# educating-dip/diffusion_models_dev_project

Hardware: NVIDIA B200
Metric: SCD samples/sec at 256^2 (higher is better)
Workload: dtype f32

## Files before the change

bench_support/adm_unet.py:

```python
import math

import torch
import torch.nn as nn
import torch.nn.functional as F


def sinusoidal_embedding(t, dim, max_period=10000.0):
    half = dim // 2
    freqs = torch.exp(-math.log(max_period) * torch.arange(half, dtype=torch.float32, device=t.device) / half)
    args = t[:, None].float() * freqs[None]
    return torch.cat([torch.cos(args), torch.sin(args)], dim=-1)


def _norm(ch):
    return nn.GroupNorm(32, ch)


def _small_init(conv, std=0.02):
    nn.init.normal_(conv.weight, std=std)
    nn.init.zeros_(conv.bias)
    return conv


class Res(nn.Module):
    def __init__(self, cin, cout, emb_ch, resample=None):
        super().__init__()
        self.resample = resample
        self.n1 = _norm(cin)
        self.c1 = nn.Conv2d(cin, cout, 3, padding=1)
        self.emb = nn.Linear(emb_ch, 2 * cout)
        self.n2 = _norm(cout)
        self.c2 = _small_init(nn.Conv2d(cout, cout, 3, padding=1))
        self.skip = nn.Identity() if cin == cout else nn.Conv2d(cin, cout, 1)

    def _rs(self, v):
        if self.resample == 'up':
            return F.interpolate(v, scale_factor=2, mode='nearest')
        if self.resample == 'down':
            return F.avg_pool2d(v, 2)
        return v

    def forward(self, x, emb):
        h = F.silu(self.n1(x))
        if self.resample is not None:
            h, x = self._rs(h), self._rs(x)
        h = self.c1(h)
        scale, shift = self.emb(F.silu(emb))[:, :, None, None].chunk(2, dim=1)
        h = self.n2(h) * (1 + scale) + shift
        h = self.c2(F.silu(h))
        return self.skip(x) + h


class Attn(nn.Module):
    def __init__(self, ch, head_ch):
        super().__init__()
        self.heads = ch // head_ch
        self.norm = _norm(ch)
        self.qkv = nn.Conv1d(ch, 3 * ch, 1)
        self.proj = _small_init(nn.Conv1d(ch, ch, 1))

    def forward(self, x, emb=None):
        b, c, hh, ww = x.shape
        q, k, v = self.qkv(self.norm(x).reshape(b, c, -1)).reshape(b * self.heads, 3 * c // self.heads, -1).chunk(3, dim=1)
        a = F.scaled_dot_product_attention(q.transpose(1, 2), k.transpose(1, 2), v.transpose(1, 2))
        a = a.transpose(1, 2).reshape(b, c, -1)
        return x + self.proj(a).reshape(b, c, hh, ww)


class Stage(nn.ModuleList):
    def forward(self, x, emb):
        for m in self:
            x = m(x, emb)
        return x


class AdmUNet(nn.Module):
    def __init__(self, image_size=256, in_channels=1, model_channels=256, out_channels=2,
                 num_res_blocks=1, channel_mult=(1, 1, 2, 2, 4, 4), attention_resolutions=(16,),
                 num_head_channels=64, max_period=1e4):
        super().__init__()
        ch = model_channels
        emb_ch = 4 * ch
        self.model_channels = ch
        self.max_period = max_period
        self.out_channels = out_channels
        self.time = nn.Sequential(nn.Linear(ch, emb_ch), nn.SiLU(), nn.Linear(emb_ch, emb_ch))
        attn_ds = {image_size // r for r in attention_resolutions}
        self.stem = nn.Conv2d(in_channels, ch, 3, padding=1)
        self.down = nn.ModuleList()
        skips = [ch]
        cur, ds = ch, 1
        for level, mult in enumerate(channel_mult):
            for _ in range(num_res_blocks):
                blk = [Res(cur, mult * ch, emb_ch)]
                cur = mult * ch
                if ds in attn_ds:
                    blk.append(Attn(cur, num_head_channels))
                self.down.append(Stage(blk)); skips.append(cur)
            if level != len(channel_mult) - 1:
                self.down.append(Stage([Res(cur, cur, emb_ch, 'down')])); skips.append(cur)
                ds *= 2
        self.mid = Stage([Res(cur, cur, emb_ch), Attn(cur, num_head_channels), Res(cur, cur, emb_ch)])
        self.up = nn.ModuleList()
        for level, mult in list(enumerate(channel_mult))[::-1]:
            for i in range(num_res_blocks + 1):
                blk = [Res(cur + skips.pop(), mult * ch, emb_ch)]
                cur = mult * ch
                if ds in attn_ds:
                    blk.append(Attn(cur, num_head_channels))
                if level and i == num_res_blocks:
                    blk.append(Res(cur, cur, emb_ch, 'up'))
                    ds //= 2
                self.up.append(Stage(blk))
        self.head = nn.Sequential(_norm(cur), nn.SiLU(), _small_init(nn.Conv2d(cur, out_channels, 3, padding=1)))

    def forward(self, x, timesteps):
        emb = self.time(sinusoidal_embedding(timesteps, self.model_channels, self.max_period))
        h = self.stem(x)
        hs = [h]
        for blk in self.down:
            h = blk(h, emb)
            hs.append(h)
        h = self.mid(h, emb)
        for blk in self.up:
            h = blk(torch.cat([h, hs.pop()], dim=1), emb)
        out = self.head(h)
        return out[:, :1] if self.out_channels == 2 else out


def small_unet():
    return AdmUNet(image_size=256, model_channels=32, out_channels=1, channel_mult=(1, 2, 4),
                   attention_resolutions=(16,), num_head_channels=32)


def aapm_unet():
    return AdmUNet()
```

diffusion_models_dev_project_b200/_lib.py:

```python
import ctypes as C
import os
import threading

_HERE = os.path.dirname(os.path.abspath(__file__))
LIB_PATH = os.environ.get("SCD_B200_LIB") or os.path.join(_HERE, "_lib", "libscd_b200.so")

SCD_E_INVALID = -10001
SCD_E_NODEVICE = -10002
SCD_E_WORKSPACE = -10003


class GeomDesc(C.Structure):
    _fields_ = [
        ("n0", C.c_int32), ("n1", C.c_int32),
        ("x_min", C.c_double), ("y_min", C.c_double), ("dx", C.c_double),
        ("n_angles", C.c_int32), ("angles", C.POINTER(C.c_double)),
        ("n_det", C.c_int32), ("s_min", C.c_double), ("ds", C.c_double),
        ("adj_scale", C.c_double),
    ]


_F = C.c_void_p
SIGNATURES = {
    "scd_geom_create": (C.c_int, [C.POINTER(GeomDesc), C.POINTER(C.c_void_p)]),
    "scd_geom_destroy": (C.c_int, [C.c_void_p]),
    "scd_fp_scratch_bytes": (C.c_size_t, [C.c_void_p, C.c_int]),
    "scd_fp": (C.c_int, [C.c_void_p, _F, _F, C.c_int, C.c_int, C.c_int, C.c_void_p, C.c_size_t, C.c_void_p]),
    "scd_bp_scratch_bytes": (C.c_size_t, [C.c_void_p, C.c_int]),
    "scd_bp": (C.c_int, [C.c_void_p, _F, _F, C.c_int, C.c_int, C.c_int, C.c_float, _F, C.c_float,
                         C.c_void_p, C.c_size_t, C.c_void_p]),
    "scd_sino_il_buffer_bytes": (C.c_size_t, [C.c_void_p, C.c_int]),
    "scd_fp_il": (C.c_int, [C.c_void_p, _F, _F, C.c_int, C.c_int, C.c_int, C.c_void_p, C.c_size_t, C.c_void_p]),
    "scd_bp_il": (C.c_int, [C.c_void_p, _F, _F, C.c_int, C.c_int, C.c_int, C.c_float, _F, C.c_float, C.c_void_p]),
    "scd_img_il_bytes": (C.c_size_t, [C.c_void_p, C.c_int]),
    "scd_img_il_pack": (C.c_int, [C.c_void_p, _F, _F, C.c_int, C.c_void_p]),
    "scd_img_il_unpack": (C.c_int, [C.c_void_p, _F, _F, C.c_int, C.c_void_p]),
    "scd_fp_ilimg": (C.c_int, [C.c_void_p, _F, _F, C.c_int, C.c_int, C.c_int, C.c_void_p]),
    "scd_bp_ilimg": (C.c_int, [C.c_void_p, _F, _F, C.c_int, C.c_int, C.c_int, C.c_float, _F, C.c_float, C.c_void_p]),
    "scd_cg_workspace_bytes": (C.c_size_t, [C.c_void_p, C.c_int]),
    "scd_cg": (C.c_int, [C.c_void_p, _F, _F, C.c_double, C.c_int, C.c_int, C.c_void_p, C.c_size_t, C.c_void_p]),
    "scd_tweedie_rhs": (C.c_int, [_F, _F, _F, _F, _F, C.c_int, C.c_double, _F, _F, C.c_int, C.c_int64, C.c_void_p]),
    "scd_ddim": (C.c_int, [_F, _F, _F, _F, _F, _F, C.c_int, C.c_double, _F, C.c_int, C.c_int64, C.c_void_p]),
    "scd_dds_step": (C.c_int, [C.c_void_p, _F, _F, _F, _F, _F, _F, _F, C.c_int, C.c_double, C.c_double,
                               C.c_int, _F, _F, C.c_int, C.c_void_p, C.c_size_t, C.c_void_p]),
    "scd_residual_sq_blocks": (C.c_int, [C.c_int64]),
    "scd_residual_sq": (C.c_int, [_F, _F, _F, _F, C.c_int64, C.c_void_p]),
    "scd_tv_blocks": (C.c_int, [C.c_int, C.c_int]),
    "scd_tv_loss": (C.c_int, [_F, _F, C.c_int, C.c_int, C.c_int, C.c_void_p]),
    "scd_tv_grad": (C.c_int, [_F, _F, C.c_int, C.c_int, C.c_int, C.c_void_p]),
    "scd_adapt_workspace_bytes": (C.c_size_t, [C.c_void_p, C.c_int, C.c_int]),
    "scd_adapt_fwd": (C.c_int, [C.c_void_p, _F, _F, _F, _F, _F, _F, C.c_int, C.c_double, C.c_int, C.c_int, C.c_double,
                                _F, _F, C.c_int, C.c_void_p, C.c_size_t, C.c_void_p]),
    "scd_adapt_bwd": (C.c_int, [C.c_void_p, _F, _F, _F, C.c_int, C.c_double, C.c_int, C.c_int, C.c_double, C.c_double,
                                _F, C.c_int, C.c_void_p, C.c_size_t, C.c_void_p]),
    "scd_ramp_filter": (C.c_int, [C.c_void_p, _F, _F, C.c_int, C.c_void_p]),
    "scd_bp_banded": (C.c_int, [C.c_void_p, _F, C.c_int, C.c_int, C.c_int, C.c_float, C.POINTER(C.c_void_p), C.c_int, C.c_int,
                                C.c_void_p, C.c_size_t, C.c_void_p]),
    "scd_bp_il_banded": (C.c_int, [C.c_void_p, _F, C.c_int, C.c_int, C.c_int, C.c_float, C.POINTER(C.c_void_p), C.c_int, C.c_int,
                                   C.c_void_p]),
    "scd_band_reduce": (C.c_int, [_F, C.c_int, C.c_int64, C.c_int, C.c_int, C.c_int, C.c_int, C.c_int, C.c_int,
                                  C.POINTER(C.c_void_p), C.c_int, C.c_int, _F, C.c_float, C.c_float, C.c_void_p]),
    "scd_fp_host": (C.c_int, [C.c_void_p, C.c_void_p, C.c_void_p, C.c_int]),
    "scd_bp_host": (C.c_int, [C.c_void_p, C.c_void_p, C.c_void_p, C.c_int]),
    "scd_geom_info": (C.c_int, [C.c_void_p, C.POINTER(C.c_int32), C.POINTER(C.c_int32),
                                C.POINTER(C.c_int32), C.POINTER(C.c_int32)]),
    "scd_launch_count": (C.c_int64, []),
    "scd_launch_count_reset": (None, []),
    "scd_set_tuning": (C.c_int, [C.c_void_p, C.c_char_p, C.c_int]),
    "scd_last_error_string": (C.c_char_p, []),
    "scd_version": (C.c_char_p, []),
}

_lib = None
_lock = threading.Lock()


def load():
    global _lib
    if _lib is not None:
        return _lib
    with _lock:
        if _lib is not None:
            return _lib
        if not os.path.exists(LIB_PATH):
            raise RuntimeError(
                f"{LIB_PATH} not found. Build it with `python -m diffusion_models_dev_project_b200.build` "
                "(needs nvcc). This package has no CPU or PyTorch fallback for the ray transform.")
        try:
            lib = C.CDLL(LIB_PATH)
        except OSError as e:
            raise RuntimeError(f"cannot load {LIB_PATH}: {e}") from e
        for name, (res, args) in SIGNATURES.items():
            fn = getattr(lib, name)
            fn.restype = res
            fn.argtypes = args
        _lib = lib
    return _lib


def last_error():
    s = load().scd_last_error_string()
    return s.decode() if s else ""


def check(rc, what):
    if rc != 0:
        raise RuntimeError(f"{what} failed (code {rc}): {last_error()}")
```

diffusion_models_dev_project_b200/build.py:

```python
import os
import shutil
import subprocess
import sys

HERE = os.path.dirname(os.path.abspath(__file__))
ROOT = os.path.dirname(HERE)
CSRC = os.path.join(HERE, "csrc")
LIB_DIR = os.path.join(HERE, "_lib")
LIB_PATH = os.path.join(LIB_DIR, "libscd_b200.so")
DEBUG_LIB_PATH = os.path.join(LIB_DIR, "libscd_b200_dbg.so")
SOURCES = ["geometry.cu", "fp_march.cu", "bp_tile.cu", "vec_ops.cu", "il_ops.cu", "loss_ops.cu", "adapt_ops.cu", "fbp_filter.cu", "cg_solver.cu", "peer_reduce.cu"]
HEADERS = [os.path.join(CSRC, "scd_internal.cuh"), os.path.join(ROOT, "include", "scd_b200.h")]
ARCH = ["-gencode", "arch=compute_100a,code=sm_100a"]


def _nvcc():
    cand = shutil.which("nvcc") or "/usr/local/cuda/bin/nvcc"
    if not os.path.exists(cand):
        raise RuntimeError("nvcc not found: libscd_b200.so cannot be built (there is no CPU fallback)")
    return cand


def needs_build(path=LIB_PATH):
    if not os.path.exists(path):
        return True
    t = os.path.getmtime(path)
    deps = [os.path.join(CSRC, s) for s in SOURCES] + HEADERS
    return any(os.path.getmtime(d) > t for d in deps)


def build(force=False, verbose=False, debug=False):
    out = DEBUG_LIB_PATH if debug else LIB_PATH
    if not force and not needs_build(out):
        return out
    os.makedirs(LIB_DIR, exist_ok=True)
    cmd = [_nvcc(), "-shared", "-Xcompiler", "-fPIC", "-O3", "-std=c++17", "-lineinfo", *ARCH,
           "-I", os.path.join(ROOT, "include"), "-I", CSRC]
    if debug:
        cmd += ["-DSCD_DEBUG_STAMPS"]
    if verbose:
        cmd += ["-Xptxas", "-v"]
    cmd += [os.path.join(CSRC, s) for s in SOURCES] + ["-o", out + ".tmp"]
    res = subprocess.run(cmd, capture_output=True, text=True)
    if res.returncode != 0:
        raise RuntimeError("nvcc failed:\n" + res.stdout + res.stderr)
    if verbose:
        sys.stderr.write(res.stdout + res.stderr)
    os.replace(out + ".tmp", out)
    return out


if __name__ == "__main__":
    p = build(force="--force" in sys.argv, verbose="--verbose" in sys.argv, debug="--debug" in sys.argv)
    print(p)
```

diffusion_models_dev_project_b200/fused.py:

```python
import ctypes as C

import torch
from torch import Tensor

from . import _lib


def _stream(device):
    return C.c_void_p(torch.cuda.current_stream(device).cuda_stream)


def _check_cuda_f32(**tensors):
    dev = None
    for name, t in tensors.items():
        if t is None:
            continue
        if not t.is_cuda:
            raise RuntimeError('%s must be a CUDA tensor (no CPU fallback in libscd_b200)' % name)
        if t.dtype != torch.float32:
            raise TypeError('%s must be float32, got %s' % (name, t.dtype))
        dev = dev or t.device
        if t.device != dev:
            raise ValueError('%s is on %s, expected %s' % (name, t.device, dev))
    return dev


def _times(t: Tensor, batch: int, device) -> Tensor:
    t = t.to(device=device, dtype=torch.float32).reshape(-1).contiguous()
    if t.numel() != batch:
        raise ValueError('time step tensor must have one entry per sample (%d != %d)' % (t.numel(), batch))
    return t


def tweedie_rhs(x: Tensor, s: Tensor, t: Tensor, abar: Tensor, atb: Tensor = None, gamma: float = 0.0):
    dev = _check_cuda_f32(x=x, s=s, atb=atb, abar=abar)
    x = x.contiguous(); s = s.contiguous()
    if s.shape != x.shape:
        raise ValueError('x %r and s %r differ in shape' % (tuple(x.shape), tuple(s.shape)))
    batch = x.shape[0]
    numel = x[0].numel()
    t = _times(t, batch, dev)
    xhat0 = torch.empty_like(x)
    b = None
    atb_ptr = None
    if atb is not None:
        atb = atb.expand_as(x).contiguous()
        b = torch.empty_like(x)
        atb_ptr = atb.data_ptr()
    lib = _lib.load()
    with torch.cuda.device(dev):
        _lib.check(lib.scd_tweedie_rhs(x.data_ptr(), s.data_ptr(), atb_ptr, t.data_ptr(), abar.data_ptr(),
                                       int(abar.numel()), float(gamma), xhat0.data_ptr(),
                                       b.data_ptr() if b is not None else None, batch, numel, _stream(dev)),
                   'scd_tweedie_rhs')
    return (xhat0, b) if atb is not None else xhat0


def ddim_ddpm(xhat: Tensor, s: Tensor, eps: Tensor, t: Tensor, t_prev: Tensor, abar: Tensor, eta: float):
    dev = _check_cuda_f32(xhat=xhat, s=s, eps=eps, abar=abar)
    xhat = xhat.contiguous(); s = s.contiguous(); eps = eps.contiguous()
    if s.shape != xhat.shape or eps.shape != xhat.shape:
        raise ValueError('xhat, s and eps must have the same shape')
    batch = xhat.shape[0]
    numel = xhat[0].numel()
    t = _times(t, batch, dev)
    t_prev = _times(t_prev, batch, dev)
    out = torch.empty_like(xhat)
    lib = _lib.load()
    with torch.cuda.device(dev):
        _lib.check(lib.scd_ddim(xhat.data_ptr(), s.data_ptr(), eps.data_ptr(), t.data_ptr(), t_prev.data_ptr(),
                                abar.data_ptr(), int(abar.numel()), float(eta), out.data_ptr(), batch, numel,
                                _stream(dev)), 'scd_ddim')
    return out


def launch_count(reset=False):
    lib = _lib.load()
    n = int(lib.scd_launch_count())
    if reset:
        lib.scd_launch_count_reset()
    return n
```

include/scd_b200.h:

```cpp
#ifndef SCD_B200_H
#define SCD_B200_H

#include <stddef.h>
#include <stdint.h>

#ifdef __cplusplus
extern "C" {
#endif

#define SCD_E_INVALID   (-10001)
#define SCD_E_NODEVICE  (-10002)
#define SCD_E_WORKSPACE (-10003)

typedef struct scd_geom scd_geom_t;

typedef struct scd_geom_desc {
    int32_t n0, n1;
    double  x_min, y_min;
    double  dx;
    int32_t n_angles;
    const double *angles;
    int32_t n_det;
    double  s_min;
    double  ds;
    double  adj_scale;
} scd_geom_desc;

int scd_geom_create(const scd_geom_desc *desc, scd_geom_t **out);
int scd_geom_destroy(scd_geom_t *g);

size_t scd_fp_scratch_bytes(const scd_geom_t *g, int batch);
int scd_fp(const scd_geom_t *g, const float *img, float *sino, int batch,
           int angle_lo, int angle_hi, void *scratch, size_t scratch_bytes,
           void *stream);

size_t scd_bp_scratch_bytes(const scd_geom_t *g, int batch);
int scd_bp(const scd_geom_t *g, const float *sino, float *out, int batch,
           int angle_lo, int angle_hi, float c_acc, const float *addend,
           float c_add, void *scratch, size_t scratch_bytes, void *stream);

size_t scd_sino_il_buffer_bytes(const scd_geom_t *g, int batch);
int scd_fp_il(const scd_geom_t *g, const float *img, float *sino_il, int batch,
              int angle_lo, int angle_hi, void *scratch, size_t scratch_bytes, void *stream);
int scd_bp_il(const scd_geom_t *g, const float *sino_il, float *out, int batch,
              int angle_lo, int angle_hi, float c_acc, const float *addend, float c_add,
              void *stream);

size_t scd_img_il_bytes(const scd_geom_t *g, int batch);
int scd_img_il_pack(const scd_geom_t *g, const float *img, float *img_il, int batch, void *stream);
int scd_img_il_unpack(const scd_geom_t *g, const float *img_il, float *img, int batch, void *stream);
int scd_fp_ilimg(const scd_geom_t *g, const float *img_il, float *sino_il, int batch,
                 int angle_lo, int angle_hi, void *stream);
int scd_bp_ilimg(const scd_geom_t *g, const float *sino_il, float *out_il, int batch,
                 int angle_lo, int angle_hi, float c_acc, const float *addend_il, float c_add, void *stream);

size_t scd_cg_workspace_bytes(const scd_geom_t *g, int batch);

int scd_cg(const scd_geom_t *g, float *x, const float *rhs, double gamma,
           int n_iter, int batch, void *work, size_t work_bytes, void *stream);


int scd_tweedie_rhs(const float *x, const float *s, const float *atb,
                    const float *t, const float *abar, int n_table,
                    double gamma, float *xhat0, float *b, int batch,
                    int64_t numel_per_sample, void *stream);

int scd_ddim(const float *xhat, const float *s, const float *eps,
             const float *t, const float *t_prev, const float *abar,
             int n_table, double eta, float *out, int batch,
             int64_t numel_per_sample, void *stream);

int scd_dds_step(const scd_geom_t *g, const float *x, const float *s,
                 const float *atb, const float *eps, const float *t,
                 const float *t_prev, const float *abar, int n_table,
                 double gamma, double eta, int n_iter, float *x_next,
                 float *xhat0, int batch, void *work, size_t work_bytes,
                 void *stream);

int scd_residual_sq_blocks(int64_t numel);
int scd_residual_sq(const float *ax, const float *y, float *r, float *part, int64_t numel, void *stream);
int scd_tv_blocks(int n0, int n1);
int scd_tv_loss(const float *x, float *part, int images, int n0, int n1, void *stream);
int scd_tv_grad(const float *x, float *grad, int images, int n0, int n1, void *stream);

size_t scd_adapt_workspace_bytes(const scd_geom_t *g, int batch, int n_iter);
int scd_adapt_fwd(const scd_geom_t *g, const float *x, const float *s, const float *atb, const float *y,
                  const float *t, const float *abar, int n_table, double gamma, int n_iter, int dc_type,
                  double tv_lambda, float *loss, float *xhat_out, int batch, void *work, size_t work_bytes,
                  void *stream);
int scd_adapt_bwd(const scd_geom_t *g, const float *grad_loss, const float *t, const float *abar, int n_table,
                  double gamma, int n_iter, int dc_type, double tv_lambda, double trafo_grad_scale,
                  float *grad_s, int batch, void *work, size_t work_bytes, void *stream);

int scd_ramp_filter(const scd_geom_t *g, const float *sino, float *out, int batch, void *stream);

int scd_bp_banded(const scd_geom_t *g, const float *sino, int batch, int angle_lo, int angle_hi,
                  float c_acc, float *const *band_ptrs, int n_bands, int band_rows,
                  void *scratch, size_t scratch_bytes, void *stream);
int scd_bp_il_banded(const scd_geom_t *g, const float *sino_il, int batch, int angle_lo, int angle_hi,
                     float c_acc, float *const *band_ptrs, int n_bands, int band_rows, void *stream);
int scd_band_reduce(const float *stage, int n_src, int64_t slot_stride_floats, int batch, int band_rows,
                    int rows, int n1, int row_lo, int n0, float *const *out_ptrs, int n_out,
                    int out_is_multicast, const float *addend, float c_add, float c_sum, void *stream);

int scd_fp_host(const scd_geom_t *g, const float *img_host, float *sino_host,
                int batch);
int scd_bp_host(const scd_geom_t *g, const float *sino_host, float *img_host,
                int batch);

int scd_geom_info(const scd_geom_t *g, int32_t *n0, int32_t *n1,
                  int32_t *n_angles, int32_t *n_det);
int64_t scd_launch_count(void);
void    scd_launch_count_reset(void);
int scd_set_tuning(scd_geom_t *g, const char *key, int value);

const char *scd_last_error_string(void);
const char *scd_version(void);

#ifdef __cplusplus
}
#endif
#endif
```

Baseline: 1.340.

## Run UNet inference in channels_last with fused GroupNorm and residual kernels

Adds an inference-only path for the ADM UNet that keeps activations in channels_last layout. It introduces custom CUDA kernels for GroupNorm (two-pass Welford statistics folded with conv bias, FiLM scale/shift and SiLU into one per-channel affine apply) and for bias-plus-residual add. Conv weights are cached in channels_last, padded to multiples of 4 channels. The goal is to cut the many separate elementwise and norm kernels and layout conversions per block, at the cost of extra layout copies around concat, resample and attention.

```diff
diff --git a/bench_support/adm_unet.py b/bench_support/adm_unet.py
--- a/bench_support/adm_unet.py
+++ b/bench_support/adm_unet.py
@@ -3,6 +3,10 @@
 import torch
 import torch.nn as nn
 import torch.nn.functional as F
+
+from diffusion_models_dev_project_b200 import fused
+
+CL = torch.channels_last
 
 
 def sinusoidal_embedding(t, dim, max_period=10000.0):
@@ -14,6 +18,54 @@
 
 def _norm(ch):
     return nn.GroupNorm(32, ch)
+
+
+def _fused_path(x):
+    return x.is_cuda and not torch.is_grad_enabled()
+
+
+def _cl(t):
+    return torch.empty_like(t, memory_format=CL).copy_(t)
+
+
+def _cl_params(conv):
+    w, b = conv.weight, conv.bias
+    key = (w.device, w.data_ptr(), w._version, None if b is None else (b.data_ptr(), b._version))
+    held = conv.__dict__.get('_cl_params')
+    if held is None or held[0] != key:
+        pad = -w.shape[0] % 4 if conv.groups == 1 else 0
+        wp, bp = w.detach(), None
+        if pad:
+            wp = torch.cat([wp, wp.new_zeros(pad, *wp.shape[1:])])
+            bp = torch.cat([b.detach(), b.new_zeros(pad)]) if b is not None else None
+        held = (key, _cl(wp), bp)
+        conv.__dict__['_cl_params'] = held
+    return held[1], held[2]
+
+
+def _conv(conv, x, add_bias):
+    if type(conv) is not nn.Conv2d or conv.padding_mode != 'zeros':
+        return conv(x).contiguous(memory_format=CL), None
+    w, b_padded = _cl_params(conv)
+    args = (conv.stride, conv.padding, conv.dilation, conv.groups)
+    if w.shape[0] != conv.out_channels:
+        y = F.conv2d(x, w, b_padded, *args)[:, :conv.out_channels]
+        return y.contiguous(memory_format=CL), None
+    y = F.conv2d(x, w, conv.bias if add_bias else None, *args)
+    return y.contiguous(memory_format=CL), (None if add_bias else conv.bias)
+
+
+def _conv1x1(conv, x, add_bias):
+    if type(conv) is not nn.Conv1d or conv.kernel_size != (1,):
+        b, c, hh, ww = x.shape
+        return conv(x.reshape(b, c, hh * ww)).reshape(b, -1, hh, ww).contiguous(memory_format=CL), None
+    y = F.conv2d(x, conv.weight[..., None], conv.bias if add_bias else None)
+    return y.contiguous(memory_format=CL), (None if add_bias else conv.bias)
+
+
+def _gn(norm, x, silu, conv_bias=None, scale_shift=None):
+    return fused.group_norm_nhwc(x, norm.num_groups, norm.weight, norm.bias, norm.eps, conv_bias=conv_bias,
+                                 scale_shift=scale_shift, silu=silu)
 
 
 def _small_init(conv, std=0.02):
@@ -41,6 +93,8 @@
         return v
 
     def forward(self, x, emb):
+        if _fused_path(x):
+            return self._forward_fused(x, emb)
         h = F.silu(self.n1(x))
         if self.resample is not None:
             h, x = self._rs(h), self._rs(x)
@@ -50,6 +104,16 @@
         h = self.c2(F.silu(h))
         return self.skip(x) + h
 
+    def _forward_fused(self, x, emb):
+        h = _gn(self.n1, x, silu=True)
+        if self.resample is not None:
+            h, x = self._rs(h).contiguous(memory_format=CL), self._rs(x).contiguous(memory_format=CL)
+        h, b1 = _conv(self.c1, h, add_bias=False)
+        h = _gn(self.n2, h, silu=True, conv_bias=b1, scale_shift=self.emb(F.silu(emb)))
+        h, b2 = _conv(self.c2, h, add_bias=False)
+        skip = x if isinstance(self.skip, nn.Identity) else _conv(self.skip, x, add_bias=True)[0]
+        return fused.residual_add_nhwc(skip, h, b2)
+
 
 class Attn(nn.Module):
     def __init__(self, ch, head_ch):
@@ -60,11 +124,24 @@
         self.proj = _small_init(nn.Conv1d(ch, ch, 1))
 
     def forward(self, x, emb=None):
+        if _fused_path(x):
+            return self._forward_fused(x)
         b, c, hh, ww = x.shape
         q, k, v = self.qkv(self.norm(x).reshape(b, c, -1)).reshape(b * self.heads, 3 * c // self.heads, -1).chunk(3, dim=1)
         a = F.scaled_dot_product_attention(q.transpose(1, 2), k.transpose(1, 2), v.transpose(1, 2))
         a = a.transpose(1, 2).reshape(b, c, -1)
         return x + self.proj(a).reshape(b, c, hh, ww)
+
+    def _forward_fused(self, x):
+        b, c, hh, ww = x.shape
+        d = c // self.heads
+        qkv, _ = _conv1x1(self.qkv, _gn(self.norm, x, silu=False), add_bias=True)
+        qkv = qkv.permute(0, 2, 3, 1).reshape(b, hh * ww, self.heads, 3, d)
+        q, k, v = (qkv[:, :, :, i].transpose(1, 2).reshape(b * self.heads, hh * ww, d) for i in range(3))
+        a = F.scaled_dot_product_attention(q, k, v)
+        a = a.reshape(b, self.heads, hh, ww, d).permute(0, 2, 3, 1, 4).reshape(b, hh, ww, c).permute(0, 3, 1, 2)
+        h, bias = _conv1x1(self.proj, a, add_bias=False)
+        return fused.residual_add_nhwc(x, h, bias)
 
 
 class Stage(nn.ModuleList):
@@ -116,6 +193,8 @@
 
     def forward(self, x, timesteps):
         emb = self.time(sinusoidal_embedding(timesteps, self.model_channels, self.max_period))
+        if _fused_path(x):
+            return self._forward_fused(x, emb)
         h = self.stem(x)
         hs = [h]
         for blk in self.down:
@@ -127,6 +206,19 @@
         out = self.head(h)
         return out[:, :1] if self.out_channels == 2 else out
 
+    def _forward_fused(self, x, emb):
+        h = _conv(self.stem, _cl(x), add_bias=True)[0]
+        hs = [h]
+        for blk in self.down:
+            h = blk(h, emb)
+            hs.append(h)
+        h = self.mid(h, emb)
+        for blk in self.up:
+            h = blk(torch.cat([h, hs.pop()], dim=1).contiguous(memory_format=CL), emb)
+        norm, _, conv = self.head
+        out = _conv(conv, _gn(norm, h, silu=True), add_bias=True)[0]
+        return out[:, :1] if self.out_channels == 2 else out
+
 
 def small_unet():
     return AdmUNet(image_size=256, model_channels=32, out_channels=1, channel_mult=(1, 2, 4),
diff --git a/diffusion_models_dev_project_b200/_lib.py b/diffusion_models_dev_project_b200/_lib.py
--- a/diffusion_models_dev_project_b200/_lib.py
+++ b/diffusion_models_dev_project_b200/_lib.py
@@ -60,6 +60,11 @@
                                    C.c_void_p]),
     "scd_band_reduce": (C.c_int, [_F, C.c_int, C.c_int64, C.c_int, C.c_int, C.c_int, C.c_int, C.c_int, C.c_int,
                                   C.POINTER(C.c_void_p), C.c_int, C.c_int, _F, C.c_float, C.c_float, C.c_void_p]),
+    "scd_gn_workspace_bytes": (C.c_size_t, [C.c_int, C.c_int, C.c_int, C.c_int]),
+    "scd_gn_stats": (C.c_int, [_F, _F, _F, _F, _F, C.c_double, C.c_int, C.c_int, C.c_int, C.c_int, _F, C.c_void_p,
+                               C.c_size_t, C.c_void_p]),
+    "scd_gn_apply": (C.c_int, [_F, _F, _F, C.c_int, C.c_int, C.c_int, C.c_int, C.c_void_p]),
+    "scd_residual_add": (C.c_int, [_F, _F, _F, _F, C.c_int64, C.c_int, C.c_void_p]),
     "scd_fp_host": (C.c_int, [C.c_void_p, C.c_void_p, C.c_void_p, C.c_int]),
     "scd_bp_host": (C.c_int, [C.c_void_p, C.c_void_p, C.c_void_p, C.c_int]),
     "scd_geom_info": (C.c_int, [C.c_void_p, C.POINTER(C.c_int32), C.POINTER(C.c_int32),
diff --git a/diffusion_models_dev_project_b200/build.py b/diffusion_models_dev_project_b200/build.py
--- a/diffusion_models_dev_project_b200/build.py
+++ b/diffusion_models_dev_project_b200/build.py
@@ -9,7 +9,7 @@
 LIB_DIR = os.path.join(HERE, "_lib")
 LIB_PATH = os.path.join(LIB_DIR, "libscd_b200.so")
 DEBUG_LIB_PATH = os.path.join(LIB_DIR, "libscd_b200_dbg.so")
-SOURCES = ["geometry.cu", "fp_march.cu", "bp_tile.cu", "vec_ops.cu", "il_ops.cu", "loss_ops.cu", "adapt_ops.cu", "fbp_filter.cu", "cg_solver.cu", "peer_reduce.cu"]
+SOURCES = ["geometry.cu", "fp_march.cu", "bp_tile.cu", "vec_ops.cu", "il_ops.cu", "loss_ops.cu", "adapt_ops.cu", "fbp_filter.cu", "cg_solver.cu", "peer_reduce.cu", "unet_ops.cu"]
 HEADERS = [os.path.join(CSRC, "scd_internal.cuh"), os.path.join(ROOT, "include", "scd_b200.h")]
 ARCH = ["-gencode", "arch=compute_100a,code=sm_100a"]
 
diff --git a/diffusion_models_dev_project_b200/csrc/unet_ops.cu b/diffusion_models_dev_project_b200/csrc/unet_ops.cu
--- /dev/null
+++ b/diffusion_models_dev_project_b200/csrc/unet_ops.cu
@@ -0,0 +1,277 @@
+#include "scd_internal.cuh"
+
+#define GN_TARGET_CTAS (148 * 8)
+#define GN_MAX_TILES   1024
+#define GN_UNROLL      4
+#define EW_THREADS     256
+
+namespace {
+
+struct GnPlan {
+    int rows;
+    int threads;
+    int tile_pix;
+    int tiles;
+};
+
+GnPlan gn_plan(int batch, int hw, int channels)
+{
+    GnPlan p;
+    const int c4 = channels / 4;
+    p.rows = c4 >= 256 ? 1 : 256 / c4;
+    p.threads = (c4 * p.rows + 31) & ~31;
+    int64_t per = ((int64_t)hw * batch + GN_TARGET_CTAS - 1) / GN_TARGET_CTAS;
+    const int64_t floor_tiles = ((int64_t)hw + GN_MAX_TILES - 1) / GN_MAX_TILES;
+    if (per < floor_tiles) per = floor_tiles;
+    if (per < 4 * p.rows) per = 4 * p.rows;
+    per = (per + p.rows - 1) / p.rows * p.rows;
+    if (per > hw) per = hw;
+    p.tile_pix = (int)per;
+    p.tiles = (int)(((int64_t)hw + per - 1) / per);
+    return p;
+}
+
+__device__ __forceinline__ void chan_merge(float &n, float &m, float &M, float nb, float mb, float Mb)
+{
+    if (nb == 0.f) return;
+    if (n == 0.f) { n = nb; m = mb; M = Mb; return; }
+    const float nn = n + nb, d = mb - m, f = nb / nn;
+    m = fmaf(d, f, m);
+    M = M + Mb + d * d * n * f;
+    n = nn;
+}
+
+__device__ __forceinline__ void chan_warp(float &n, float &m, float &M)
+{
+    const int lane = threadIdx.x & 31;
+#pragma unroll
+    for (int off = 16; off > 0; off >>= 1) {
+        const float nb = __shfl_down_sync(0xffffffffu, n, off);
+        const float mb = __shfl_down_sync(0xffffffffu, m, off);
+        const float Mb = __shfl_down_sync(0xffffffffu, M, off);
+        if (lane + off < 32) chan_merge(n, m, M, nb, mb, Mb);
+    }
+}
+
+__device__ __forceinline__ void welford4(float4 &m, float4 &M, float inv, float4 v)
+{
+    float d;
+    d = v.x - m.x; m.x = fmaf(d, inv, m.x); M.x = fmaf(d, v.x - m.x, M.x);
+    d = v.y - m.y; m.y = fmaf(d, inv, m.y); M.y = fmaf(d, v.y - m.y, M.y);
+    d = v.z - m.z; m.z = fmaf(d, inv, m.z); M.z = fmaf(d, v.z - m.z, M.z);
+    d = v.w - m.w; m.w = fmaf(d, inv, m.w); M.w = fmaf(d, v.w - m.w, M.w);
+}
+
+__device__ __forceinline__ float4 add4(float4 a, float4 b)
+{
+    return make_float4(a.x + b.x, a.y + b.y, a.z + b.z, a.w + b.w);
+}
+
+__global__ void __launch_bounds__(1024)
+gn_stats_kernel(const float *__restrict__ x, const float *__restrict__ bias, int hw, int C, int G, int rows,
+                int tile_pix, int tiles, float2 *__restrict__ part)
+{
+    extern __shared__ float sm[];
+    scd_pdl_wait();
+    scd_pdl_trigger();
+    const int n = blockIdx.y, t = blockIdx.x, C4 = C >> 2;
+    const int q = threadIdx.x % C4, r = threadIdx.x / C4;
+    const int p_lo = t * tile_pix, p_hi = min(hw, p_lo + tile_pix);
+    float4 m = make_float4(0.f, 0.f, 0.f, 0.f), M = m;
+    if (r < rows) {
+        const float4 *x4 = reinterpret_cast<const float4 *>(x) + (size_t)n * hw * C4 + q;
+        const float4 bv = bias ? reinterpret_cast<const float4 *>(bias)[q] : make_float4(0.f, 0.f, 0.f, 0.f);
+        int k = 0, p = p_lo + r;
+        for (; p + (GN_UNROLL - 1) * rows < p_hi; p += GN_UNROLL * rows) {
+            float4 v[GN_UNROLL];
+#pragma unroll
+            for (int u = 0; u < GN_UNROLL; ++u) v[u] = x4[(size_t)(p + u * rows) * C4];
+#pragma unroll
+            for (int u = 0; u < GN_UNROLL; ++u) { ++k; welford4(m, M, 1.f / (float)k, add4(v[u], bv)); }
+        }
+        for (; p < p_hi; p += rows) { ++k; welford4(m, M, 1.f / (float)k, add4(x4[(size_t)p * C4], bv)); }
+        float *sm_m = sm + r * C + 4 * q, *sm_M = sm + rows * C + r * C + 4 * q;
+        sm_m[0] = m.x; sm_m[1] = m.y; sm_m[2] = m.z; sm_m[3] = m.w;
+        sm_M[0] = M.x; sm_M[1] = M.y; sm_M[2] = M.z; sm_M[3] = M.w;
+    }
+    __syncthreads();
+    const int cpg = C / G, items = rows * cpg, lane = threadIdx.x & 31, nw = blockDim.x >> 5;
+    for (int g = threadIdx.x >> 5; g < G; g += nw) {
+        float cn = 0.f, cm = 0.f, cM = 0.f;
+        for (int i = lane; i < items; i += 32) {
+            const int rr = i / cpg, c = g * cpg + i % cpg;
+            const int cnt = max(0, (p_hi - p_lo - rr + rows - 1) / rows);
+            chan_merge(cn, cm, cM, (float)cnt, sm[rr * C + c], sm[rows * C + rr * C + c]);
+        }
+        chan_warp(cn, cm, cM);
+        if (lane == 0) part[((size_t)n * tiles + t) * G + g] = make_float2(cm, cM);
+    }
+}
+
+__global__ void __launch_bounds__(256)
+gn_finalize_kernel(const float2 *__restrict__ part, int hw, int C, int G, int tile_pix, int tiles,
+                   const float *__restrict__ gamma, const float *__restrict__ beta, const float *__restrict__ bias,
+                   const float *__restrict__ ss, float eps, float *__restrict__ ab)
+{
+    __shared__ float2 stat[1024];
+    scd_pdl_wait();
+    scd_pdl_trigger();
+    const int n = blockIdx.x, cpg = C / G, lane = threadIdx.x & 31;
+    for (int g = threadIdx.x >> 5; g < G; g += blockDim.x >> 5) {
+        float cn = 0.f, cm = 0.f, cM = 0.f;
+        for (int t = lane; t < tiles; t += 32) {
+            const float2 pv = part[((size_t)n * tiles + t) * G + g];
+            const int cnt = (min(hw, (t + 1) * tile_pix) - t * tile_pix) * cpg;
+            chan_merge(cn, cm, cM, (float)cnt, pv.x, pv.y);
+        }
+        chan_warp(cn, cm, cM);
+        if (lane == 0) stat[g] = make_float2(cm, rsqrtf(fmaxf(cM / cn, 0.f) + eps));
+    }
+    __syncthreads();
+    for (int c = threadIdx.x; c < C; c += blockDim.x) {
+        const float2 st = stat[c / cpg];
+        float a = st.y * gamma[c];
+        float b = fmaf(-a, st.x, beta[c]);
+        if (ss) {
+            const float s1 = 1.f + ss[(size_t)n * 2 * C + c];
+            a = a * s1;
+            b = fmaf(b, s1, ss[(size_t)n * 2 * C + C + c]);
+        }
+        if (bias) b = fmaf(a, bias[c], b);
+        ab[(size_t)n * 2 * C + c] = a;
+        ab[(size_t)n * 2 * C + C + c] = b;
+    }
+}
+
+__device__ __forceinline__ float silu_f(float v) { return v / (1.f + expf(-v)); }
+
+template <bool SILU>
+__global__ void __launch_bounds__(EW_THREADS)
+gn_apply_kernel(const float4 *x, const float *__restrict__ ab, float4 *y, int64_t total4, int64_t per4, int C4)
+{
+    scd_pdl_wait();
+    scd_pdl_trigger();
+    for (int64_t i = (int64_t)blockIdx.x * EW_THREADS + threadIdx.x; i < total4; i += (int64_t)gridDim.x * EW_THREADS) {
+        const int64_t n = i / per4;
+        const int q = (int)((i - n * per4) % C4);
+        const float4 *ab4 = reinterpret_cast<const float4 *>(ab) + n * 2 * C4;
+        const float4 a = __ldg(ab4 + q), b = __ldg(ab4 + C4 + q);
+        float4 v = x[i];
+        v.x = fmaf(a.x, v.x, b.x); v.y = fmaf(a.y, v.y, b.y); v.z = fmaf(a.z, v.z, b.z); v.w = fmaf(a.w, v.w, b.w);
+        if (SILU) { v.x = silu_f(v.x); v.y = silu_f(v.y); v.z = silu_f(v.z); v.w = silu_f(v.w); }
+        y[i] = v;
+    }
+}
+
+__global__ void __launch_bounds__(EW_THREADS)
+residual_kernel(const float4 *skip, const float4 *h, const float *__restrict__ bias, float4 *out, int64_t total4, int C4)
+{
+    scd_pdl_wait();
+    scd_pdl_trigger();
+    for (int64_t i = (int64_t)blockIdx.x * EW_THREADS + threadIdx.x; i < total4; i += (int64_t)gridDim.x * EW_THREADS) {
+        const float4 s = skip[i];
+        float4 v = h[i];
+        if (bias) {
+            const float4 b = __ldg(reinterpret_cast<const float4 *>(bias) + (int)(i % C4));
+            v.x = __fadd_rn(v.x, b.x); v.y = __fadd_rn(v.y, b.y); v.z = __fadd_rn(v.z, b.z); v.w = __fadd_rn(v.w, b.w);
+        }
+        v.x = __fadd_rn(s.x, v.x); v.y = __fadd_rn(s.y, v.y); v.z = __fadd_rn(s.z, v.z); v.w = __fadd_rn(s.w, v.w);
+        out[i] = v;
+    }
+}
+
+inline bool aligned16(const void *p) { return ((uintptr_t)p & 15) == 0; }
+
+int ew_blocks(int64_t total4)
+{
+    const int64_t want = (total4 + EW_THREADS - 1) / EW_THREADS, cap = 148 * 8;
+    return (int)(want < cap ? (want > 0 ? want : 1) : cap);
+}
+
+}
+
+extern "C" size_t scd_gn_workspace_bytes(int batch, int hw, int channels, int groups)
+{
+    if (batch <= 0 || hw <= 0 || channels <= 0 || groups <= 0) return 0;
+    const GnPlan p = gn_plan(batch, hw, channels);
+    return (size_t)batch * p.tiles * groups * sizeof(float2);
+}
+
+extern "C" int scd_gn_stats(const float *x, const float *bias, const float *gamma, const float *beta,
+                            const float *scale_shift, double eps, int batch, int hw, int channels, int groups,
+                            float *ab, void *work, size_t work_bytes, void *stream)
+{
+    if (!x || !gamma || !beta || !ab || !work) { scd_set_error("scd_gn_stats: null argument"); return SCD_E_INVALID; }
+    if (batch <= 0 || hw <= 0 || channels <= 0 || groups <= 0 || channels % 4 || channels % groups
+        || channels > 4096 || groups > 1024 || batch > 65535) {
+        scd_set_error("scd_gn_stats: unsupported shape batch %d, hw %d, channels %d, groups %d (channels must be a "
+                      "multiple of 4 and of groups, at most 4096)", batch, hw, channels, groups);
+        return SCD_E_INVALID;
+    }
+    if (!aligned16(x) || (bias && !aligned16(bias))) {
+        scd_set_error("scd_gn_stats: x and bias must be 16-byte aligned"); return SCD_E_INVALID;
+    }
+    if (work_bytes < scd_gn_workspace_bytes(batch, hw, channels, groups)) {
+        scd_set_error("scd_gn_stats: workspace of %zu bytes, need %zu", work_bytes,
+                      scd_gn_workspace_bytes(batch, hw, channels, groups));
+        return SCD_E_WORKSPACE;
+    }
+    const GnPlan p = gn_plan(batch, hw, channels);
+    cudaStream_t st = (cudaStream_t)stream;
+    float2 *part = reinterpret_cast<float2 *>(work);
+    const size_t smem = (size_t)2 * p.rows * channels * sizeof(float);
+    SCD_CUDA(scd_launch_kernel(gn_stats_kernel, dim3(p.tiles, batch), dim3(p.threads), smem, st, 0,
+                               x, bias, hw, channels, groups, p.rows, p.tile_pix, p.tiles, part));
+    SCD_LAUNCH_CHECK("gn_stats_kernel");
+    SCD_CUDA(scd_launch_kernel(gn_finalize_kernel, dim3(batch), dim3(256), 0, st, 0,
+                               (const float2 *)part, hw, channels, groups, p.tile_pix, p.tiles, gamma, beta, bias,
+                               scale_shift, (float)eps, ab));
+    SCD_LAUNCH_CHECK("gn_finalize_kernel");
+    return 0;
+}
+
+extern "C" int scd_gn_apply(const float *x, const float *ab, float *y, int batch, int hw, int channels, int silu,
+                            void *stream)
+{
+    if (!x || !ab || !y) { scd_set_error("scd_gn_apply: null argument"); return SCD_E_INVALID; }
+    if (batch <= 0 || hw <= 0 || channels <= 0 || channels % 4) {
+        scd_set_error("scd_gn_apply: unsupported shape batch %d, hw %d, channels %d", batch, hw, channels);
+        return SCD_E_INVALID;
+    }
+    if (!aligned16(x) || !aligned16(ab) || !aligned16(y)) {
+        scd_set_error("scd_gn_apply: x, ab and y must be 16-byte aligned"); return SCD_E_INVALID;
+    }
+    const int C4 = channels / 4;
+    const int64_t per4 = (int64_t)hw * C4, total4 = per4 * batch;
+    cudaStream_t st = (cudaStream_t)stream;
+    const float4 *x4 = reinterpret_cast<const float4 *>(x);
+    float4 *y4 = reinterpret_cast<float4 *>(y);
+    if (silu)
+        SCD_CUDA(scd_launch_kernel(gn_apply_kernel<true>, dim3(ew_blocks(total4)), dim3(EW_THREADS), 0, st, 0,
+                                   x4, ab, y4, total4, per4, C4));
+    else
+        SCD_CUDA(scd_launch_kernel(gn_apply_kernel<false>, dim3(ew_blocks(total4)), dim3(EW_THREADS), 0, st, 0,
+                                   x4, ab, y4, total4, per4, C4));
+    SCD_LAUNCH_CHECK("gn_apply_kernel");
+    return 0;
+}
+
+extern "C" int scd_residual_add(const float *skip, const float *h, const float *bias, float *out, int64_t pixels,
+                                int channels, void *stream)
+{
+    if (!skip || !h || !out) { scd_set_error("scd_residual_add: null argument"); return SCD_E_INVALID; }
+    if (pixels <= 0 || channels <= 0 || channels % 4) {
+        scd_set_error("scd_residual_add: unsupported shape pixels %lld, channels %d", (long long)pixels, channels);
+        return SCD_E_INVALID;
+    }
+    if (!aligned16(skip) || !aligned16(h) || !aligned16(out) || (bias && !aligned16(bias))) {
+        scd_set_error("scd_residual_add: buffers must be 16-byte aligned"); return SCD_E_INVALID;
+    }
+    const int C4 = channels / 4;
+    const int64_t total4 = pixels * C4;
+    SCD_CUDA(scd_launch_kernel(residual_kernel, dim3(ew_blocks(total4)), dim3(EW_THREADS), 0, (cudaStream_t)stream, 0,
+                               reinterpret_cast<const float4 *>(skip), reinterpret_cast<const float4 *>(h), bias,
+                               reinterpret_cast<float4 *>(out), total4, C4));
+    SCD_LAUNCH_CHECK("residual_kernel");
+    return 0;
+}
diff --git a/diffusion_models_dev_project_b200/fused.py b/diffusion_models_dev_project_b200/fused.py
--- a/diffusion_models_dev_project_b200/fused.py
+++ b/diffusion_models_dev_project_b200/fused.py
@@ -74,6 +74,55 @@
     return out
 
 
+def _nhwc(name, x: Tensor):
+    if x.dim() != 4 or not x.is_contiguous(memory_format=torch.channels_last):
+        raise ValueError('%s must be a 4-D channels_last tensor, got shape %r strides %r'
+                         % (name, tuple(x.shape), x.stride()))
+
+
+def _per_channel(name, v: Tensor, c: int):
+    if v is not None and (v.shape != (c,) or not v.is_contiguous()):
+        raise ValueError('%s must be a contiguous [%d] tensor, got %r' % (name, c, tuple(v.shape)))
+
+
+def group_norm_nhwc(x: Tensor, groups: int, weight: Tensor, bias: Tensor, eps: float = 1e-5,
+                    conv_bias: Tensor = None, scale_shift: Tensor = None, silu: bool = False) -> Tensor:
+    dev = _check_cuda_f32(x=x, weight=weight, bias=bias, conv_bias=conv_bias, scale_shift=scale_shift)
+    _nhwc('x', x)
+    n, c, h, w = x.shape
+    _per_channel('weight', weight, c); _per_channel('bias', bias, c); _per_channel('conv_bias', conv_bias, c)
+    if scale_shift is not None and (scale_shift.shape != (n, 2 * c) or not scale_shift.is_contiguous()):
+        raise ValueError('scale_shift must be a contiguous [%d, %d] tensor, got %r' % (n, 2 * c, tuple(scale_shift.shape)))
+    lib = _lib.load()
+    ab = torch.empty(n, 2 * c, device=dev, dtype=torch.float32)
+    work = torch.empty(int(lib.scd_gn_workspace_bytes(n, h * w, c, groups)), device=dev, dtype=torch.uint8)
+    y = torch.empty_like(x)
+    ptr = lambda t: t.data_ptr() if t is not None else None
+    with torch.cuda.device(dev):
+        st = _stream(dev)
+        _lib.check(lib.scd_gn_stats(x.data_ptr(), ptr(conv_bias), weight.data_ptr(), bias.data_ptr(), ptr(scale_shift),
+                                    float(eps), n, h * w, c, int(groups), ab.data_ptr(), work.data_ptr(), work.numel(),
+                                    st), 'scd_gn_stats')
+        _lib.check(lib.scd_gn_apply(x.data_ptr(), ab.data_ptr(), y.data_ptr(), n, h * w, c, int(bool(silu)), st),
+                   'scd_gn_apply')
+    return y
+
+
+def residual_add_nhwc(skip: Tensor, h: Tensor, bias: Tensor = None) -> Tensor:
+    dev = _check_cuda_f32(skip=skip, h=h, bias=bias)
+    _nhwc('skip', skip); _nhwc('h', h)
+    if skip.shape != h.shape:
+        raise ValueError('skip %r and h %r differ in shape' % (tuple(skip.shape), tuple(h.shape)))
+    n, c, hh, ww = h.shape
+    _per_channel('bias', bias, c)
+    out = torch.empty_like(h)
+    lib = _lib.load()
+    with torch.cuda.device(dev):
+        _lib.check(lib.scd_residual_add(skip.data_ptr(), h.data_ptr(), bias.data_ptr() if bias is not None else None,
+                                        out.data_ptr(), n * hh * ww, c, _stream(dev)), 'scd_residual_add')
+    return out
+
+
 def launch_count(reset=False):
     lib = _lib.load()
     n = int(lib.scd_launch_count())
diff --git a/include/scd_b200.h b/include/scd_b200.h
--- a/include/scd_b200.h
+++ b/include/scd_b200.h
@@ -103,6 +103,15 @@
                     int rows, int n1, int row_lo, int n0, float *const *out_ptrs, int n_out,
                     int out_is_multicast, const float *addend, float c_add, float c_sum, void *stream);
 
+size_t scd_gn_workspace_bytes(int batch, int hw, int channels, int groups);
+int scd_gn_stats(const float *x, const float *bias, const float *gamma, const float *beta,
+                 const float *scale_shift, double eps, int batch, int hw, int channels, int groups,
+                 float *ab, void *work, size_t work_bytes, void *stream);
+int scd_gn_apply(const float *x, const float *ab, float *y, int batch, int hw, int channels, int silu,
+                 void *stream);
+int scd_residual_add(const float *skip, const float *h, const float *bias, float *out, int64_t pixels,
+                     int channels, void *stream);
+
 int scd_fp_host(const scd_geom_t *g, const float *img_host, float *sino_host,
                 int batch);
 int scd_bp_host(const scd_geom_t *g, const float *sino_host, float *img_host,
```

New measurement: 2.207, median of 6. +64.7%, better.
